# hyeeiin/ECG-Multimodal-Model

Measured on AMD Instinct MI355X. Metric: samples/sec fwd+bwd, batch-256 multimodal (img+sig+clin), 1->8 MI355X, higher is better.
Workload: dtype bf16; 1 GPU; full multimodal (image 3x224x224 + 5000-pt signal + 16-dim clinical), fwd+bwd+Adam, encoders unfrozen; image_hw=224x224, per_gpu_batch=256, global_batch=256, parallelism=dp1

## Files before the change

### ecg-multimodal-model_amd/csrc/api.hip

```cpp
#include <stdarg.h>

#include "ops.h"

static thread_local char g_err[512] = "";

void ecg_set_error(const char* fmt, ...) {
  va_list ap;
  va_start(ap, fmt);
  vsnprintf(g_err, sizeof(g_err), fmt, ap);
  va_end(ap);
}

static inline ConvGeom geom_of(const ecgmm_conv_desc* c) {
  return make_geom(c->N, c->H, c->W, c->Cin, c->Cout, c->R, c->S, c->stride, c->pad_h, c->pad_w);
}
#define S_(x) ((hipStream_t)(x))

extern "C" {

int ecgmm_version(void) { return ECGMM_VERSION; }
const char* ecgmm_last_error(void) { return g_err; }

const char* ecgmm_switch_name(int i) { return i >= 0 && i < sw::COUNT ? sw::ALL[i]->env : nullptr; }
int ecgmm_switch_get(const char* env_name, int64_t* value) {
// ... 251 lines not shown
  if (c->N < 1 || c->H < 1 || c->W < 1 || c->Cin < 1 || c->Cout < 1 || c->R < 1 || c->S < 1 || c->stride < 1 ||
      c->pad_h < 0 || c->pad_w < 0 || c->H + 2 * c->pad_h < c->R || c->W + 2 * c->pad_w < c->S)
    ECG_FAIL(ECGMM_ERR_SHAPE, "conv_fwd_fused: bad geometry");
  return ecg_conv_igemm(dtype, 0, geom_of(c), x, w_fwd, y, bias, addend, nullptr, act, S_(stream));
}
int ecgmm_fold_conv_bn(int dtype, int layout, const float* w, const float* conv_bias, const float* gamma, const float* beta,
                       const float* running_mean, const float* running_var, float eps, void* w_out, float* b_out,
                       float* scale_out, int Cout, int Cin, int RS, void* stream) {
  if (layout != 0 && layout != 1) ECG_FAIL(ECGMM_ERR_SHAPE, "fold_conv_bn: layout %d (0 = forward pack, 1 = stem pack)", layout);
  EcgFoldItem it = {};
  it.kind = layout == 1 ? ECG_FOLD_STEM : ECG_FOLD_CONV;
  it.w = w; it.conv_bias = conv_bias; it.gamma = gamma; it.beta = beta; it.rm = running_mean; it.rv = running_var;
  it.wout = w_out; it.bout = b_out; it.scale_out = scale_out; it.Cout = Cout; it.Cin = Cin; it.RS = RS;
  return ecg_fold_batch(dtype, &it, 1, eps, S_(stream));
}
int ecgmm_relu_maxpool(int dtype, const void* y, void* out, int N, int H, int W, int C, void* stream) {
  return ecg_relu_maxpool(dtype, y, out, N, H, W, C, S_(stream));
}
int ecgmm_gate_res_relu(int dtype, const void* y, const float* gate, const void* res, void* out, int64_t M, int C,
                        int rows_per_sample, void* stream) {
  return ecg_gate_res_relu(dtype, y, gate, res, out, (long)M, C, rows_per_sample, S_(stream));
}

int ecgmm_avgpool(int dtype, const void* x, float* out, int N, int R, int C, const float* coef, void* stream) {
  return ecg_avgpool(dtype, x, out, N, R, C, coef, S_(stream));
}
int ecgmm_bcast_rows(int dtype, const float* v, void* out, int N, int R, int C, float scale, void* stream) {
  return ecg_bcast_rows(dtype, v, out, N, R, C, scale, S_(stream));
}
int ecgmm_se_gate_grad(int dtype, const void* dout, const void* maskref, const void* y, const float* coef, float* dg,
                       int N, int R, int C, void* stream) {
  return ecg_se_gate_grad(dtype, dout, maskref, y, coef, dg, N, R, C, S_(stream));
}

static int se_mlp_shape(const char* what, int N, int C, int CR) {
  if (N < 1 || C < 1 || C > 1024 || CR < 1 || CR > 64)
    ECG_FAIL(ECGMM_ERR_SHAPE, "%s: N=%d C=%d CR=%d outside N >= 1, C 1..1024, CR 1..64", what, N, C, CR);
  return 0;
}
int ecgmm_se_mlp_fwd(const float* m, const float* w1, const float* b1, const float* w2, const float* b2, float* h, float* g,
                     int N, int C, int CR, void* stream) {
  ECG_TRY(se_mlp_shape("se_mlp_fwd", N, C, CR));
  return ecg_se_mlp_fwd(m, w1, b1, w2, b2, h, g, N, C, CR, S_(stream));
}
int ecgmm_se_mlp_bwd(const float* dg, const float* g, const float* h, const float* m, const float* w1, const float* w2,
                     float* ds, float* dh, float* dm, float* dw1, float* db1, float* dw2, float* db2, int N, int C, int CR,
                     float scale, void* stream) {
  ECG_TRY(se_mlp_shape("se_mlp_bwd", N, C, CR));
  return ecg_se_mlp_bwd(dg, g, h, m, w1, w2, ds, dh, dm, dw1, db1, dw2, db2, N, C, CR, scale, S_(stream));
}

int ecgmm_linear_fwd(const float* x, const float* w, const float* bias, float* y, int B, int In, int Out, int act,
                     void* stream) {
  return ecg_linear_fwd(x, w, bias, y, B, In, Out, act, nullptr, S_(stream));
}
size_t ecgmm_linear_bwd_scratch(int B, int In, int Out) { return ecg_linear_bwd_scratch(B, In, Out); }
int ecgmm_linear_bwd(const float* dz, const float* x, const float* w, float* dx, float* dw, float* db, int B, int In,
                     int Out, void* scratch, size_t scratch_bytes, void* stream) {
  return ecg_linear_bwd(dz, x, w, dx, dw, db, B, In, Out, scratch, scratch_bytes, S_(stream));
}
int ecgmm_act_bwd(const float* dy, const float* y, float* dz, int64_t n, int act, void* stream) {
  return ecg_act_bwd(dy, y, dz, (long)n, act, S_(stream));
}

int ecgmm_layernorm_fwd(const float* const* seg, const int* dims, int nseg, const float* fusion_w, const float* gamma,
                        const float* beta, float* out, float* stat, float* soft_w, int B, float eps, void* stream) {
// ... 98 lines not shown
```

### ecg-multimodal-model_amd/csrc/elementwise.hip

```cpp
#include "ops.h"

namespace {

constexpr int EW_THREADS = 256;

__device__ __forceinline__ u32x4 ld16(const void* p) { return *reinterpret_cast<const u32x4*>(p); }
__device__ __forceinline__ u32x4 ld16s(const void* p) {
#ifndef EW_NO_NT
  return __builtin_nontemporal_load(reinterpret_cast<const u32x4*>(p));
#else
  return *reinterpret_cast<const u32x4*>(p);
#endif
}
struct RowDiv { unsigned mul, sh; };
__device__ __forceinline__ long row_div(long r, RowDiv d) { return (long)(((unsigned long long)(unsigned)r * d.mul) >> d.sh); }
static RowDiv make_row_div(int d) {
  unsigned dd = d < 1 ? 1u : (unsigned)d;
  int l = 0;
  while ((1u << l) < dd) ++l;
  RowDiv r;
  r.mul = (unsigned)(((1ull << (31 + l)) + dd - 1) / dd);
  r.sh = 31u + (unsigned)l;
  return r;
}
// ... 673 lines not shown
    if (dgamma) dgamma[c] = (float)s2;
    if (dbeta) dbeta[c] = (float)s1;
    bcoef[c] = (gamma ? gamma[c] : 1.f) * coef[3 * C + c];
    bcoef[C + c] = (float)(s1 / count);
    bcoef[2 * C + c] = (float)(s2 / count);
  }
}

__global__ __launch_bounds__(1024) void rows_sum_kernel(const float* __restrict__ partial, int rows, int C, float* out,
                                                        int accumulate) {
  __shared__ double sh[16][64];
  const int c = blockIdx.x * 64 + (threadIdx.x & 63);
  const int slice = threadIdx.x >> 6;
  double s = 0.0;
  if (c < C) {
    int r = slice;
    for (; r + 48 < rows; r += 64) {
      float a[4];
#pragma unroll
      for (int u = 0; u < 4; ++u) a[u] = partial[(size_t)(r + 16 * u) * C + c];
#pragma unroll
      for (int u = 0; u < 4; ++u) s += (double)a[u];
    }
    for (; r < rows; r += 16) s += (double)partial[(size_t)r * C + c];
  }
  sh[slice][threadIdx.x & 63] = s;
  __syncthreads();
  if (slice == 0 && c < C) {
    for (int k = 1; k < 16; ++k) s += sh[k][threadIdx.x];
    out[c] = accumulate ? out[c] + (float)s : (float)s;
  }
}

template <typename T>
__global__ __launch_bounds__(EW_THREADS) void bnrelu_maxpool_kernel(const T* __restrict__ y,
                                                                    const float* __restrict__ coef, T* __restrict__ out,
                                                                    unsigned char* __restrict__ idx, int N, int H,
                                                                    int W, int C, int OH, int OW) {
  constexpr int VEC = Elem<T>::VEC;
  const int cpr = C / VEC;
  long total = (long)N * OH * OW * cpr;
  for (long i = (long)blockIdx.x * blockDim.x + threadIdx.x; i < total; i += (long)gridDim.x * blockDim.x) {
    int chunk = (int)(i % cpr);
    long pix = i / cpr;
    int ow = (int)(pix % OW);
    long t = pix / OW;
    int oh = (int)(t % OH), n = (int)(t / OH);
    int c0 = chunk * VEC;
    float best[VEC];
    int bi[VEC];
    if constexpr (sizeof(T) == 2) {
      unsigned key[VEC];
      float scv[VEC], shv[VEC];
#pragma unroll
      for (int j = 0; j < VEC; ++j) {
        key[j] = 0u;
        scv[j] = coef[c0 + j];
        shv[j] = coef[C + c0 + j];
      }
#pragma unroll
      for (int kh = 0; kh < 3; ++kh) {
        int h = oh * 2 - 1 + kh;
        if ((unsigned)h >= (unsigned)H) continue;
#pragma unroll
        for (int kw = 0; kw < 3; ++kw) {
          int w = ow * 2 - 1 + kw;
          if ((unsigned)w >= (unsigned)W) continue;
          float f[VEC];
          unpack16<T>(ld16(y + (((size_t)n * H + h) * W + w) * C + c0), f);
#pragma unroll
          for (int j = 0; j < VEC; ++j) f[j] = fmaxf(f[j] * scv[j] + shv[j], 0.f);
          const u32x4 r = pack16<bf16_t>(f);
          const unsigned tcode = 15u - (unsigned)(kh * 3 + kw);
#pragma unroll
          for (int q = 0; q < 4; ++q) {
            key[2 * q] = max(key[2 * q], ((r[q] & 0x7fffu) << 4) | tcode);
            key[2 * q + 1] = max(key[2 * q + 1], (((r[q] >> 16) & 0x7fffu) << 4) | tcode);
          }
        }
      }
#pragma unroll
      for (int j = 0; j < VEC; ++j) {
        best[j] = __uint_as_float((key[j] >> 4) << 16);
        bi[j] = 15 - (int)(key[j] & 15u);
      }
    } else {
#pragma unroll
      for (int j = 0; j < VEC; ++j) {
        best[j] = -INFINITY;
        bi[j] = 0;
      }
#pragma unroll
      for (int kh = 0; kh < 3; ++kh) {
        int h = oh * 2 - 1 + kh;
        if ((unsigned)h >= (unsigned)H) continue;
#pragma unroll
        for (int kw = 0; kw < 3; ++kw) {
          int w = ow * 2 - 1 + kw;
          if ((unsigned)w >= (unsigned)W) continue;
          float f[VEC];
          unpack16<T>(ld16(y + (((size_t)n * H + h) * W + w) * C + c0), f);
#pragma unroll
          for (int j = 0; j < VEC; ++j) {
            float a = fmaxf(f[j] * coef[c0 + j] + coef[C + c0 + j], 0.f);
            if (a > best[j]) {
              best[j] = a;
              bi[j] = kh * 3 + kw;
            }
          }
        }
      }
    }
    st16(out + pix * C + c0, pack16<T>(best));
    unsigned pk[VEC / 4];
#pragma unroll
    for (int q = 0; q < VEC / 4; ++q)
      pk[q] = (unsigned)bi[4 * q] | ((unsigned)bi[4 * q + 1] << 8) | ((unsigned)bi[4 * q + 2] << 16) |
              ((unsigned)bi[4 * q + 3] << 24);
    unsigned* ip = reinterpret_cast<unsigned*>(idx + pix * C + c0);
    if constexpr (VEC == 8) *reinterpret_cast<uint2*>(ip) = make_uint2(pk[0], pk[1]);
    else ip[0] = pk[0];
  }
}

template <typename T>
__global__ __launch_bounds__(EW_THREADS) void maxpool_relu_bwd_kernel(const T* __restrict__ dp,
                                                                      const T* __restrict__ pooled,
                                                                      const unsigned char* __restrict__ idx,
                                                                      T* __restrict__ dz, int N, int H, int W, int C,
                                                                      int OH, int OW) {
  constexpr int VEC = Elem<T>::VEC;
  const int cpr = C / VEC;
  const int H2 = (H + 1) >> 1, W2 = (W + 1) >> 1;
  long total = (long)N * H2 * W2 * cpr;
  for (long i = (long)blockIdx.x * blockDim.x + threadIdx.x; i < total; i += (long)gridDim.x * blockDim.x) {
    int chunk = (int)(i % cpr);
    long blk = i / cpr;
    int m = (int)(blk % W2);
    long t = blk / W2;
    int k = (int)(t % H2), n = (int)(t / H2);
    int c0 = chunk * VEC;
    float d[4][VEC], pv[4][VEC];
    unsigned pk[4][2];
    bool wok[4];
#pragma unroll
    for (int a = 0; a < 2; ++a)
#pragma unroll
      for (int b = 0; b < 2; ++b) {
        const int q = a * 2 + b;
        wok[q] = k + a < OH && m + b < OW;
        const size_t o = (((size_t)n * OH + (wok[q] ? k + a : k)) * OW + (wok[q] ? m + b : m)) * C + c0;
        unpack16<T>(ld16(dp + o), d[q]);
        unpack16<T>(ld16(pooled + o), pv[q]);
        if constexpr (VEC == 8) {
// ... 178 lines not shown
  }
  if (partial) {
#pragma unroll
    for (int j = 0; j < VEC; ++j) shm[threadIdx.x][j] = a1[j];
    __syncthreads();
    for (int c = threadIdx.x; c < C; c += POOL_THREADS) {
      int ck = c / VEC, j = c % VEC;
      float sum = 0.f;
      for (int k = 0; k < bpi; ++k) sum += shm[k * cpr + ck][j];
      partial[(size_t)blockIdx.x * C + c] = sum;
    }
  }
}

template <typename T, bool SEGATE>
__global__ __launch_bounds__(EW_THREADS) void sample_reduce_kernel(const T* __restrict__ x,
                                                                   const T* __restrict__ maskref,
                                                                   const T* __restrict__ y,
                                                                   const float* __restrict__ coef,
                                                                   float* __restrict__ out, int R, int C) {
  constexpr int VEC = Elem<T>::VEC;
  __shared__ float sh[EW_THREADS][VEC + 1];
  const int cpr = C / VEC, nsl = EW_THREADS / cpr;
  const int chunk = threadIdx.x % cpr, slice = threadIdx.x / cpr;
  const int n = blockIdx.x, c0 = chunk * VEC;
  float acc[VEC], sc[VEC], sf[VEC];
#pragma unroll
  for (int j = 0; j < VEC; ++j) {
    acc[j] = 0.f;
    sc[j] = (SEGATE || coef) ? coef[c0 + j] : 1.f;
    sf[j] = (SEGATE || coef) ? coef[C + c0 + j] : 0.f;
  }
  int r = slice;
  if (!SEGATE) {
    for (; r + 3 * nsl < R; r += 4 * nsl) {
      u32x4 q[4];
#pragma unroll
      for (int u = 0; u < 4; ++u) q[u] = ld16(x + ((size_t)n * R + r + u * nsl) * C + c0);
#pragma unroll
      for (int u = 0; u < 4; ++u) {
        float f[VEC];
        unpack16<T>(q[u], f);
#pragma unroll
        for (int j = 0; j < VEC; ++j) acc[j] += f[j];
      }
    }
  }
  for (; r < R; r += nsl) {
    const size_t o = ((size_t)n * R + r) * C + c0;
    float f[VEC];
    unpack16<T>(ld16(x + o), f);
    if (SEGATE) {
      float m[VEC], v[VEC];
      unpack16<T>(ld16(maskref + o), m);
      unpack16<T>(ld16(y + o), v);
#pragma unroll
      for (int j = 0; j < VEC; ++j)
        if (m[j] > 0.f) acc[j] += f[j] * (v[j] * sc[j] + sf[j]);
    } else {
#pragma unroll
      for (int j = 0; j < VEC; ++j) acc[j] += f[j];
    }
  }
#pragma unroll
  for (int j = 0; j < VEC; ++j) sh[threadIdx.x][j] = acc[j];
  __syncthreads();
  for (int c = threadIdx.x; c < C; c += EW_THREADS) {
    const int ck = c / VEC, j = c % VEC;
    float s_ = 0.f;
    for (int k = 0; k < nsl; ++k) s_ += sh[k * cpr + ck][j];
    if (!SEGATE) {
      s_ /= (float)R;
      if (coef) s_ = s_ * coef[c] + coef[C + c];
    }
    out[(size_t)n * C + c] = s_;
  }
}

template <typename T>
__global__ __launch_bounds__(EW_THREADS) void se_gate_bn_kernel(const T* __restrict__ dout, const T* __restrict__ maskref,
                                                                const T* __restrict__ y, const float* __restrict__ coef,
                                                                T* __restrict__ dz, float* __restrict__ dg,
                                                                float* __restrict__ a1o, float* __restrict__ a2o,
                                                                float* __restrict__ a3o, int R, int C) {
  constexpr int VEC = Elem<T>::VEC;
  __shared__ float sh[EW_THREADS][VEC + 1];
  const int cpr = C / VEC, nsl = EW_THREADS / cpr;
  const int chunk = threadIdx.x % cpr, slice = threadIdx.x / cpr;
  const int n = blockIdx.x, c0 = chunk * VEC;
  float sc[VEC], sf[VEC], mu[VEC], ag[VEC], a1[VEC], a2[VEC], a3[VEC];
#pragma unroll
  for (int j = 0; j < VEC; ++j) {
    sc[j] = coef[c0 + j];
    sf[j] = coef[C + c0 + j];
    mu[j] = coef[2 * C + c0 + j];
    ag[j] = a1[j] = a2[j] = a3[j] = 0.f;
  }
  for (int r = slice; r < R; r += nsl) {
    const size_t o = ((size_t)n * R + r) * C + c0;
    float f[VEC], m[VEC], v[VEC];
    unpack16<T>(ld16(dout + o), f);
    unpack16<T>(ld16(maskref + o), m);
    unpack16<T>(ld16(y + o), v);
#pragma unroll
    for (int j = 0; j < VEC; ++j) {
      f[j] = m[j] > 0.f ? f[j] : 0.f;
      const float yc = v[j] - mu[j];
      ag[j] += f[j] * (v[j] * sc[j] + sf[j]);
      a1[j] += f[j];
      a2[j] += f[j] * yc;
      a3[j] += yc;
    }
    st16(dz + o, pack16<T>(f));
  }
  float* const outs[4] = {dg, a1o, a2o, a3o};
#pragma unroll
  for (int q = 0; q < 4; ++q) {
#pragma unroll
    for (int j = 0; j < VEC; ++j) sh[threadIdx.x][j] = q == 0 ? ag[j] : q == 1 ? a1[j] : q == 2 ? a2[j] : a3[j];
    __syncthreads();
    for (int c = threadIdx.x; c < C; c += EW_THREADS) {
      const int ck = c / VEC, j = c % VEC;
      float s_ = 0.f;
      for (int k = 0; k < nsl; ++k) s_ += sh[k * cpr + ck][j];
      outs[q][(size_t)n * C + c] = s_;
    }
    __syncthreads();
  }
}

constexpr int SE_ROWS = 16;
__global__ __launch_bounds__(256) void se_bn_rows_kernel(const float* __restrict__ a1, const float* __restrict__ a2,
                                                         const float* __restrict__ a3, const float* __restrict__ gate,
                                                         const float* __restrict__ addc, int N, int R, int C,
                                                         float* __restrict__ rows) {
  __shared__ float sh[2][4][64];
  const int c = blockIdx.x * 64 + (threadIdx.x & 63), sl = threadIdx.x >> 6, j = blockIdx.y;
  float s1 = 0.f, s2 = 0.f;
  if (c < C)
    for (int n = j + SE_ROWS * sl; n < N; n += SE_ROWS * 4) {
      const size_t o = (size_t)n * C + c;
      const float g = gate ? gate[o] : 1.f, ad = addc ? addc[o] : 0.f;
      s1 += g * a1[o] + ad * (float)R;
      s2 += g * a2[o] + ad * a3[o];
    }
  sh[0][sl][threadIdx.x & 63] = s1;
// ... 492 lines not shown
  hipLaunchKernelGGL(bn_bwd_finalize_kernel, dim3(ceil_div(C, 64)), dim3(1024), 0, stream, (const float*)partial, g1, C,
                     (double)M, gamma, coef, dgamma, dbeta, bcoef, 1);
  ECG_CHECK_LAUNCH("bn_bwd_finalize");
  *bcoef_out = bcoef;
  return 0;
}

bool ecg_stem_fuse_on() { return sw::STEM_FUSE.get() != 0; }

int ecg_pool_bn_bwd(int dtype, const void* dp, const void* pooled, const unsigned char* idx, const void* y,
                    const float* coef, const float* gamma, float* dgamma, float* dbeta, void* dy, float* dbias, int N,
                    int H, int W, int C, float* scratch, hipStream_t stream) {
  if (!chunk_ok(C, dtype)) ECG_FAIL(ECGMM_ERR_SHAPE, "pool_bn_bwd: C=%d unsupported", C);
  const int OH = (H - 1) / 2 + 1, OW = (W - 1) / 2 + 1;
  const int rows = bn_bwd_rows(dtype, (long)N * H * W, C);
  DISPATCH_T(dtype, (pool_bwd_launch<bf16_t>(dp, pooled, idx, y, coef, gamma, dgamma, dbeta, dy, dbias, N, H, W, C, OH, OW, scratch, rows, stream)),
             (pool_bwd_launch<float>(dp, pooled, idx, y, coef, gamma, dgamma, dbeta, dy, dbias, N, H, W, C, OH, OW, scratch, rows, stream)),
             "pool_bn_bwd");
  ECG_CHECK_LAUNCH("pool_bn_bwd");
  return 0;
}

int ecg_rows_sum(const float* partial, int rows, int C, float* out, int accumulate, hipStream_t stream) {
  hipLaunchKernelGGL(rows_sum_kernel, dim3(ceil_div(C, 64)), dim3(1024), 0, stream, partial, rows, C, out, accumulate);
  ECG_CHECK_LAUNCH("rows_sum");
  return 0;
}

int ecg_bnrelu_maxpool(int dtype, const void* y, const float* coef, void* out, unsigned char* idx, int N, int H, int W,
                       int C, hipStream_t stream) {
  if (!chunk_ok(C, dtype)) ECG_FAIL(ECGMM_ERR_SHAPE, "maxpool: C=%d unsupported", C);
  int OH = (H + 2 - 3) / 2 + 1, OW = (W + 2 - 3) / 2 + 1;
  int vec = dtype == ECGMM_BF16 ? 8 : 4;
  int grid = ew_grid((long)N * OH * OW * (C / vec), EW_THREADS);
  DISPATCH_T(dtype,
             hipLaunchKernelGGL(bnrelu_maxpool_kernel<bf16_t>, dim3(grid), dim3(EW_THREADS), 0, stream,
                                (const bf16_t*)y, coef, (bf16_t*)out, idx, N, H, W, C, OH, OW),
             hipLaunchKernelGGL(bnrelu_maxpool_kernel<float>, dim3(grid), dim3(EW_THREADS), 0, stream, (const float*)y,
                                coef, (float*)out, idx, N, H, W, C, OH, OW),
             "maxpool");
  ECG_CHECK_LAUNCH("bnrelu_maxpool");
  return 0;
}

int ecg_maxpool_relu_bwd(int dtype, const void* dp, const void* pooled, const unsigned char* idx, void* dz, int N,
                         int H, int W, int C, hipStream_t stream) {
  if (!chunk_ok(C, dtype)) ECG_FAIL(ECGMM_ERR_SHAPE, "maxpool bwd: C=%d unsupported", C);
  int OH = (H + 2 - 3) / 2 + 1, OW = (W + 2 - 3) / 2 + 1;
  int vec = dtype == ECGMM_BF16 ? 8 : 4;
  int grid = ew_grid((long)N * ((H + 1) / 2) * ((W + 1) / 2) * (C / vec), EW_THREADS);
  DISPATCH_T(dtype,
             hipLaunchKernelGGL(maxpool_relu_bwd_kernel<bf16_t>, dim3(grid), dim3(EW_THREADS), 0, stream,
                                (const bf16_t*)dp, (const bf16_t*)pooled, idx, (bf16_t*)dz, N, H, W, C, OH, OW),
             hipLaunchKernelGGL(maxpool_relu_bwd_kernel<float>, dim3(grid), dim3(EW_THREADS), 0, stream,
                                (const float*)dp, (const float*)pooled, idx, (float*)dz, N, H, W, C, OH, OW),
             "maxpool bwd");
  ECG_CHECK_LAUNCH("maxpool_relu_bwd");
  return 0;
}

int ecg_avgpool(int dtype, const void* x, float* out, int N, int R, int C, const float* coef, hipStream_t stream) {
  if (!chunk_ok(C, dtype)) ECG_FAIL(ECGMM_ERR_SHAPE, "avgpool: C=%d unsupported", C);
  DISPATCH_T(dtype,
             hipLaunchKernelGGL((sample_reduce_kernel<bf16_t, false>), dim3(N), dim3(EW_THREADS), 0, stream,
                                (const bf16_t*)x, (const bf16_t*)nullptr, (const bf16_t*)nullptr, coef, out, R, C),
             hipLaunchKernelGGL((sample_reduce_kernel<float, false>), dim3(N), dim3(EW_THREADS), 0, stream,
                                (const float*)x, (const float*)nullptr, (const float*)nullptr, coef, out, R, C),
// ... 136 lines not shown
```

### ecg-multimodal-model_amd/hip/lib.py

```python
import ctypes as C
import os

F32, BF16 = 0, 1
ACT_NONE, ACT_RELU, ACT_SIGMOID = 0, 1, 2
RESNET18_NPARAMS, RESNET18_NBUFFERS = 62, 60
RESNET1D_NPARAMS, RESNET1D_NBUFFERS = 52, 27

_PKG_DIR = os.path.dirname(os.path.dirname(os.path.abspath(__file__)))
LIB_PATH = os.environ.get("ECGMM_LIB") or os.path.join(_PKG_DIR, "libecgmm_hip.so")

vp, i32, i64, u64, f32, f64, sz = C.c_void_p, C.c_int, C.c_int64, C.c_uint64, C.c_float, C.c_double, C.c_size_t


class ConvDesc(C.Structure):
    _fields_ = [(n, i32) for n in ("N", "H", "W", "Cin", "Cout", "R", "S", "stride", "pad_h", "pad_w")]


class ResNet18Desc(C.Structure):
    _fields_ = [("N", i32), ("H", i32), ("W", i32), ("out_dim", i32), ("dtype", i32), ("training", i32),
                ("bn_momentum", f32), ("bn_eps", f32)]


class ResNet1DDesc(C.Structure):
    _fields_ = [("N", i32), ("cin", i32), ("L", i32), ("num_classes", i32), ("dtype", i32), ("training", i32),
# ... 81 lines not shown
    "ecgmm_stem_bwd_weight_workspace": (sz, [i32, i32, i32, i32, i32]),
    "ecgmm_stem_bwd_weight": (i32, [i32, vp, vp, vp, i32, vp, sz, i32, i32, i32, i32, i32, vp]),
    "ecgmm_stem_bwd_data": (i32, [i32, vp, vp, vp, i32, i32, i32, i32, i32, vp]),
    "ecgmm_col_stats_rows": (i32, [i32, i64, i32]),
    "ecgmm_col_stats": (i32, [i32, vp, i64, i32, vp, vp]),
    "ecgmm_bn_finalize": (i32, [vp, i32, i32, f64, vp, vp, vp, vp, vp, f32, f32, vp, vp]),
    "ecgmm_bn_eval_coef": (i32, [i32, vp, vp, vp, vp, f32, vp, vp]),
    "ecgmm_bn_act": (i32, [i32, vp, vp, vp, vp, vp, i32, i32, vp, i64, i32, vp]),
    "ecgmm_bn_act_from_rows": (i32, [i32, vp, vp, i32, f64, vp, vp, vp, vp, vp, f32, f32, vp, vp, vp, vp, i32, i32, vp, i64, i32, vp]),
    "ecgmm_bn_bwd_scratch": (sz, [i32, i64, i32]),
    "ecgmm_bn_bwd": (i32, [i32, vp, vp, vp, vp, i32, vp, vp, vp, vp, vp, vp, vp, vp, i64, i32, vp, vp]),
    "ecgmm_bn_eval_bwd": (i32, [i32, vp, vp, vp, vp, i32, vp, vp, vp, vp, vp, vp, vp, i64, i32, vp, vp]),
    "ecgmm_conv_bwd_data_with_downsample": (i32, [i32, P(ConvDesc), vp, vp, vp, vp, vp, vp, vp]),
    "ecgmm_conv_bwd_data_bnred": (i32, [i32, P(ConvDesc), vp, vp, vp, vp, vp, vp, vp, vp, P(i32), vp]),
    "ecgmm_conv_bwd_data_bnred_rows": (i32, [i32, P(ConvDesc)]),
    "ecgmm_bn_bwd_from_rows": (i32, [i32, vp, vp, vp, vp, vp, vp, vp, vp, vp, i32, i64, i32, vp, vp]),
    "ecgmm_bnrelu_maxpool": (i32, [i32, vp, vp, vp, vp, i32, i32, i32, i32, vp]),
    "ecgmm_maxpool_relu_bwd": (i32, [i32, vp, vp, vp, vp, i32, i32, i32, i32, vp]),
    "ecgmm_bn_fuse_min_pixels": (i32, [i64]),
    "ecgmm_bn_fold": (i32, [i32]),
    "ecgmm_bn_fold_slice": (i32, [i32]),
    "ecgmm_bn_act_from_rows_bits": (i32, [i32, vp, vp, i32, f64, vp, vp, vp, vp, vp, f32, f32, vp, vp, vp, vp, i32, i32, vp, vp, i64, i32, vp]),
    "ecgmm_bn_bwd_bits": (i32, [i32, vp, vp, vp, vp, i32, vp, vp, vp, vp, vp, vp, vp, vp, i64, i32, vp, vp]),
    "ecgmm_bn_bwd_dual": (i32, [i32] + [vp] * 19 + [i64, i32, vp, vp, vp]),
    "ecgmm_bn_dual": (i32, [i32]),
    "ecgmm_tl_enable": (i32, [i32]),
    "ecgmm_tl_mark": (i32, [i32, vp]),
    "ecgmm_tl_collect": (i32, [i32, vp, vp]),
    "ecgmm_stem_recompute": (i32, [i32]),
    "ecgmm_pool_bn_bwd": (i32, [i32, vp, vp, vp, vp, vp, vp, vp, vp, vp, vp, i32, i32, i32, i32, vp, vp]),
    "ecgmm_avgpool": (i32, [i32, vp, vp, i32, i32, i32, vp, vp]),
    "ecgmm_bcast_rows": (i32, [i32, vp, vp, i32, i32, i32, f32, vp]),
    "ecgmm_se_gate_grad": (i32, [i32, vp, vp, vp, vp, vp, i32, i32, i32, vp]),
    "ecgmm_se_mlp_fwd": (i32, [vp, vp, vp, vp, vp, vp, vp, i32, i32, i32, vp]),
    "ecgmm_se_mlp_bwd": (i32, [vp, vp, vp, vp, vp, vp, vp, vp, vp, vp, vp, vp, vp, i32, i32, i32, f32, vp]),
    "ecgmm_linear_fwd": (i32, [vp, vp, vp, vp, i32, i32, i32, i32, vp]),
    "ecgmm_linear_bwd_scratch": (sz, [i32, i32, i32]),
    "ecgmm_linear_bwd": (i32, [vp, vp, vp, vp, vp, vp, i32, i32, i32, vp, sz, vp]),
    "ecgmm_act_bwd": (i32, [vp, vp, vp, i64, i32, vp]),
    "ecgmm_layernorm_fwd": (i32, [P(vp), P(i32), i32, vp, vp, vp, vp, vp, vp, i32, f32, vp]),
    "ecgmm_layernorm_bwd_scratch": (sz, [i32, i32]),
    "ecgmm_layernorm_bwd": (i32, [P(vp), P(i32), i32, vp, vp, vp, vp, P(vp), i32, vp, vp, vp, i32, vp, vp]),
    "ecgmm_varloss_fwd": (i32, [vp, vp, vp, i32, i32, i32, i32, vp, vp, vp]),
    "ecgmm_varloss_bwd": (i32, [vp, i32, i32, vp, vp, i32, vp, i32, vp]),
    "ecgmm_ce_fwd": (i32, [vp, vp, i32, i32, i32, f32, f32, vp, vp, vp]),
    "ecgmm_ce_bwd": (i32, [vp, vp, i32, i32, vp, vp, vp, vp]),
    "ecgmm_ce_plus_fwd": (i32, [vp, vp, i32, i32, vp, f32, vp, vp, vp]),
    "ecgmm_ce_plus_bwd": (i32, [vp, vp, i32, i32, vp, vp, vp, vp, f32, vp]),
    "ecgmm_dropout_fwd": (i32, [vp, vp, vp, i64, f32, u64, u64, vp]),
    "ecgmm_dropout_bwd": (i32, [vp, vp, vp, i64, f32, vp]),
    "ecgmm_adam": (i32, [vp, vp, vp, vp, i64, f32, f32, f32, f32, f32, i64, f32, vp]),
    "ecgmm_axpby": (i32, [f32, vp, f32, vp, i64, vp]),
    "ecgmm_signal_preprocess_workspace": (sz, [i32, i32, i32]),
    "ecgmm_signal_preprocess": (i32, [vp, vp, i32, i32, vp, vp, i32, P(f64), P(f64), P(f64), i32, vp, sz, vp]),
    "ecgmm_signal_preprocess_i16": (i32, [vp, i32, i32, i32, P(i32), i32, vp, vp, i32, vp, i32, i32, P(f64), P(f64), P(f64),
                                          i32, vp]),
    "ecgmm_weighted_sample": (i32, [vp, i64, i64, vp, vp, i64, u64, u64, vp]),
    "ecgmm_signal_filter_zscore": (i32, [vp, vp, i32, i32, P(f64), P(f64), P(f64), i32, i32, f64, vp]),
    "ecgmm_signal_gather_augment": (i32, [vp, i64, i32, vp, i32, vp, vp, i32, f32, f32, f32, f32, i32, i32, u64, u64, vp]),
    "ecgmm_glu_fwd": (i32, [vp, vp, i64, i32, vp]),
    "ecgmm_glu_bwd": (i32, [vp, vp, vp, i64, i32, vp]),
    "ecgmm_sparsemax_fwd": (i32, [vp, vp, i64, i32, vp]),
    "ecgmm_sparsemax_bwd": (i32, [vp, vp, vp, i64, i32, vp]),
    "ecgmm_ew": (i32, [i32, vp, vp, vp, i64, f32, vp]),
    "ecgmm_split_cols": (i32, [vp, vp, vp, i64, i32, i32, i32, vp]),
    "ecgmm_split_cols_bwd": (i32, [vp, vp, vp, vp, i64, i32, i32, i32, vp]),
# ... 48 lines not shown
    "ecgmm_shap_gradient": (i32, [vp, vp, vp, vp, vp, vp, vp, i32, i32, i32, i32, i32, i32, vp, vp, vp, vp, sz, vp]),
    "ecgmm_shap_deep": (i32, [vp, vp, vp, vp, vp, i32, i32, i32, i32, i32, vp, vp, vp, vp, sz, vp]),
    "ecgmm_mha_bwd_workspace": (sz, [P(MHADesc)]),
    "ecgmm_mha_forward": (i32, [P(MHADesc), vp, vp, vp, u64, u64, vp]),
    "ecgmm_mha_backward": (i32, [P(MHADesc), vp, vp, vp, vp, vp, vp, sz, u64, u64, vp]),
    "ecgmm_mha_keep_mask": (i32, [P(MHADesc), vp, u64, u64, vp]),
    "ecgmm_embed1d_fwd": (i32, [vp, vp, vp, vp, vp, i32, i32, i32, i32, vp]),
    "ecgmm_embed1d_bwd_workspace": (sz, [i32, i32, i32, i32]),
    "ecgmm_embed1d_bwd": (i32, [vp, vp, vp, vp, vp, vp, vp, i32, i32, i32, i32, i32, vp, sz, vp]),
}

LATER_SYMBOLS = ("ecgmm_resnet18_backward_dx", "ecgmm_resnet18_gradcam", "ecgmm_resnet1d_backward_dx",
                 "ecgmm_resnet1d_gradcam", "ecgmm_stem_bwd_data", "ecgmm_bn_eval_bwd", "ecgmm_bn_small_eval_bwd",
                 "ecgmm_resnet18_infer_prepared_bytes", "ecgmm_resnet18_infer_prepare", "ecgmm_resnet18_infer_workspace",
                 "ecgmm_resnet18_infer", "ecgmm_resnet1d_infer_prepared_bytes", "ecgmm_resnet1d_infer_prepare",
                 "ecgmm_resnet1d_infer_workspace", "ecgmm_resnet1d_infer", "ecgmm_infer_down_side", "ecgmm_conv_fwd_fused",
                 "ecgmm_fold_conv_bn", "ecgmm_relu_maxpool", "ecgmm_gate_res_relu",
                 "ecgmm_signal_filter_zscore", "ecgmm_signal_gather_augment",
                 "ecgmm_lstm_fwd_workspace", "ecgmm_lstm_bwd_workspace", "ecgmm_lstm_forward", "ecgmm_lstm_backward",
                 "ecgmm_conv5_in1_stats_rows", "ecgmm_conv5_in1_fwd", "ecgmm_conv5_in1_bwd_weight_workspace",
                 "ecgmm_conv5_in1_bwd_weight", "ecgmm_conv5_bwd_weight_workspace", "ecgmm_conv5_bwd_weight",
                 "ecgmm_bnrelu_maxpool2", "ecgmm_pool2_bn_bwd_workspace", "ecgmm_pool2_bn_bwd",
                 "ecgmm_crnn_front_fwd_workspace", "ecgmm_crnn_front_bwd_workspace", "ecgmm_crnn_front_forward",
                 "ecgmm_crnn_front_backward",
                 "ecgmm_switch_name", "ecgmm_switch_get", "ecgmm_switch_set",
                 "ecgmm_log_spectrogram_frames", "ecgmm_log_spectrogram",
                 "ecgmm_se_mlp_fwd", "ecgmm_se_mlp_bwd",
                 "ecgmm_signal_preprocess_i16", "ecgmm_weighted_sample",
                 "ecgmm_resnet18_ws_view", "ecgmm_resnet1d_ws_view",
                 "ecgmm_lime_perturb", "ecgmm_lime_ridge_workspace", "ecgmm_lime_ridge", "ecgmm_lime_prob",
                 "ecgmm_shap_mlp_workspace", "ecgmm_shap_gradient", "ecgmm_shap_deep",
                 "ecgmm_bn_bwd_dual", "ecgmm_bn_dual",
                 "ecgmm_mha_bwd_workspace", "ecgmm_mha_forward", "ecgmm_mha_backward", "ecgmm_mha_keep_mask",
                 "ecgmm_embed1d_fwd", "ecgmm_embed1d_bwd_workspace", "ecgmm_embed1d_bwd")

_lib = None


def _missing(name):
    def fail(*_a):
        raise RuntimeError(f"{LIB_PATH} does not export {name}: rebuild the HIP library (there is no fallback)")
    return fail


def lib():
    global _lib
    if _lib is None:
        if not os.path.exists(LIB_PATH):
            raise RuntimeError(
                f"libecgmm_hip.so not found at {LIB_PATH}: the HIP extension is the only compute path "
                "(no CPU fallback). Build it with `python __graft_entry__.py` or "
                "`make -C ecg-multimodal-model_amd/csrc`.")
        import torch
        h = C.CDLL(LIB_PATH)
        for name, (res, args) in SIGNATURES.items():
            if name in LATER_SYMBOLS and os.environ.get("ECGMM_LIB") and not hasattr(h, name):
                setattr(h, name, _missing(name))
                continue
            fn = getattr(h, name)
            fn.restype, fn.argtypes = res, args
        if h.ecgmm_version() != 100:
            raise RuntimeError(f"libecgmm_hip.so version {h.ecgmm_version()} != 100 (stale build?)")
        _lib = h
    return _lib


def check(rc, what=""):
# ... 4 lines not shown
```

### include/ecgmm.h

```cpp
#ifndef ECGMM_H
#define ECGMM_H
#include <stddef.h>
#include <stdint.h>

#ifdef __cplusplus
extern "C" {
#endif

#define ECGMM_VERSION 100

enum { ECGMM_F32 = 0, ECGMM_BF16 = 1 };
enum { ECGMM_ACT_NONE = 0, ECGMM_ACT_RELU = 1, ECGMM_ACT_SIGMOID = 2 };
enum {
  ECGMM_OK = 0,
  ECGMM_ERR_SHAPE = 1,
  ECGMM_ERR_DTYPE = 2,
  ECGMM_ERR_WORKSPACE = 3,
  ECGMM_ERR_LAUNCH = 4
};

int ecgmm_version(void);
const char* ecgmm_last_error(void);

const char* ecgmm_switch_name(int i);
// ... 179 lines not shown
                           const float* gamma, float* dgamma, float* dbeta, void* dy, const float* rows, int nrows,
                           int64_t M, int C, void* scratch, void* stream);

int ecgmm_bn_fuse_min_pixels(int64_t m);
int ecgmm_bn_fold(int on);
int ecgmm_bn_fold_slice(int on);
int ecgmm_bn_act_from_rows_bits(int dtype, const void* y, const float* partial, int rows, double count, const float* gamma,
                                const float* beta, float* running_mean, float* running_var, int64_t* num_batches_tracked,
                                float momentum, float eps, float* coef_out, const void* res, const float* rcoef,
                                const float* gate, int rows_per_sample, int relu, void* out, uint8_t* relu_bits, int64_t M,
                                int C, void* stream);
int ecgmm_bn_bwd_bits(int dtype, const void* dout, const uint8_t* mask_bits, const float* gate, const float* addc,
                      int rows_per_sample, const void* y, const float* coef, const float* gamma, float* dgamma,
                      float* dbeta, void* dy, void* dz_out, float* dbias, int64_t M, int C, void* scratch, void* stream);
int ecgmm_bn_bwd_dual(int dtype, const void* dout, const void* maskref, const uint8_t* mask_bits, const float* gate,
                      const float* addc, const void* y_a, const float* coef_a, const float* gamma_a, float* dgamma_a,
                      float* dbeta_a, void* dy_a, const void* y_b, const float* coef_b, const float* gamma_b,
                      float* dgamma_b, float* dbeta_b, void* dy_b, void* dz, float* dbias, int64_t M, int C, void* scratch_a,
                      void* scratch_b, void* stream);
int ecgmm_bn_dual(int on);
int ecgmm_stem_recompute(int on);

int ecgmm_bnrelu_maxpool(int dtype, const void* y, const float* coef, void* out, uint8_t* idx, int N, int H, int W,
                         int C, void* stream);
int ecgmm_maxpool_relu_bwd(int dtype, const void* dp, const void* pooled, const uint8_t* idx, void* dz, int N, int H,
                           int W, int C, void* stream);
int ecgmm_pool_bn_bwd(int dtype, const void* dp, const void* pooled, const uint8_t* idx, const void* y, const float* coef,
                      const float* gamma, float* dgamma, float* dbeta, void* dy, float* dbias, int N, int H, int W, int C,
                      void* scratch, void* stream);
int ecgmm_avgpool(int dtype, const void* x, float* out, int N, int R, int C, const float* coef, void* stream);
int ecgmm_bcast_rows(int dtype, const float* v, void* out, int N, int R, int C, float scale, void* stream);
int ecgmm_se_gate_grad(int dtype, const void* dout, const void* maskref, const void* y, const float* coef, float* dg,
                       int N, int R, int C, void* stream);
int ecgmm_se_mlp_fwd(const float* m, const float* w1, const float* b1, const float* w2, const float* b2, float* h, float* g,
                     int N, int C, int CR, void* stream);
int ecgmm_se_mlp_bwd(const float* dg, const float* g, const float* h, const float* m, const float* w1, const float* w2,
                     float* ds, float* dh, float* dm, float* dw1, float* db1, float* dw2, float* db2, int N, int C, int CR,
                     float scale, void* stream);

int ecgmm_linear_fwd(const float* x, const float* w, const float* bias, float* y, int B, int In, int Out, int act,
                     void* stream);
size_t ecgmm_linear_bwd_scratch(int B, int In, int Out);
int ecgmm_linear_bwd(const float* dz, const float* x, const float* w, float* dx, float* dw, float* db, int B, int In,
                     int Out, void* scratch, size_t scratch_bytes, void* stream);
int ecgmm_act_bwd(const float* dy, const float* y, float* dz, int64_t n, int act, void* stream);

int ecgmm_layernorm_fwd(const float* const* seg, const int* dims, int nseg, const float* fusion_w, const float* gamma,
                        const float* beta, float* out, float* stat, float* soft_w, int B, float eps, void* stream);
size_t ecgmm_layernorm_bwd_scratch(int B, int D);
int ecgmm_layernorm_bwd(const float* const* seg, const int* dims, int nseg, const float* fusion_w, const float* gamma,
                        const float* stat, const float* dout, float* const* dseg, int dseg_accumulate, float* dgamma,
                        float* dbeta, float* dfusion_w, int B, void* scratch, void* stream);

int ecgmm_varloss_fwd(const float* f0, const float* f1, const float* f2, int B, int D0, int D1, int D2, float* loss,
                      float* scratch, void* stream);
int ecgmm_varloss_bwd(const float* f, int B, int D, const float* gout, const float* scratch, int which, float* df,
                      int accumulate, void* stream);

int ecgmm_ce_fwd(const float* logits, const int64_t* labels, int B, int C, int focal, float alpha, float gamma,
                 float* loss, float* dcoef, void* stream);
int ecgmm_ce_bwd(const float* logits, const int64_t* labels, int B, int C, const float* dcoef, const float* gout,
                 float* dlogits, void* stream);
int ecgmm_ce_plus_fwd(const float* logits, const int64_t* labels, int B, int C, const float* extra, float extra_w,
                      float* loss, float* dcoef, void* stream);
int ecgmm_ce_plus_bwd(const float* logits, const int64_t* labels, int B, int C, const float* dcoef, const float* gout,
                      float* dlogits, float* dextra, float extra_w, void* stream);
// ... 145 lines not shown
```

Baseline: 40000 samples/s.

## Pool two output columns per thread and batch loads in SE gate kernels

The BN+ReLU+maxpool kernel now computes two adjacent output columns per thread from one shared 3x5 window. Overlapping input columns are loaded once, and the window is clamped and masked rather than branched. Per-channel BN coefficients are hoisted out of the grid-stride loop. The SE gate-grad and gate+BN backward kernels are unrolled by four rows with all loads issued before compute, which exposes more memory-level parallelism. A C API entry for the fused se_gate_bn kernel is also exported. Register pressure rises, and hoisting the coefficients assumes the grid stride is a multiple of cpr.

Result: faster. 40680 samples/s, median of 6 (+1.7%).

```diff
diff --git a/ecg-multimodal-model_amd/csrc/api.hip b/ecg-multimodal-model_amd/csrc/api.hip
--- a/ecg-multimodal-model_amd/csrc/api.hip
+++ b/ecg-multimodal-model_amd/csrc/api.hip
@@ -307,6 +307,12 @@
                        int N, int R, int C, void* stream) {
   return ecg_se_gate_grad(dtype, dout, maskref, y, coef, dg, N, R, C, S_(stream));
 }
+int ecgmm_se_gate_bn(int dtype, const void* dout, const void* maskref, const void* y, const float* coef, void* dz, float* dg,
+                     float* a1, float* a2, float* a3, int N, int R, int C, void* stream) {
+  if (!dout || !maskref || !y || !coef || !dz || !dg || !a1 || !a2 || !a3) ECG_FAIL(ECGMM_ERR_SHAPE, "se_gate_bn: null operand");
+  if (N < 1 || R < 1) ECG_FAIL(ECGMM_ERR_SHAPE, "se_gate_bn: N=%d R=%d", N, R);
+  return ecg_se_gate_bn(dtype, dout, maskref, y, coef, dz, dg, a1, a2, a3, N, R, C, S_(stream));
+}
 
 static int se_mlp_shape(const char* what, int N, int C, int CR) {
   if (N < 1 || C < 1 || C > 1024 || CR < 1 || CR > 64)
diff --git a/ecg-multimodal-model_amd/csrc/elementwise.hip b/ecg-multimodal-model_amd/csrc/elementwise.hip
--- a/ecg-multimodal-model_amd/csrc/elementwise.hip
+++ b/ecg-multimodal-model_amd/csrc/elementwise.hip
@@ -729,6 +729,99 @@
   }
 }
 
+template <typename T, int NR>
+__device__ __forceinline__ void pool_window2(const T* __restrict__ y, const float* scv, const float* shv, int n, int oh,
+                                             int ow0, int H, int W, int C, int c0, float (*best)[Elem<T>::VEC],
+                                             int (*bi)[Elem<T>::VEC]) {
+  constexpr int VEC = Elem<T>::VEC;
+  constexpr int KH0 = NR == 1 ? 1 : 0;
+  u32x4 q[NR * 5];
+  bool in[NR * 5];
+#pragma unroll
+  for (int kh = 0; kh < NR; ++kh) {
+    const int h = oh * 2 - 1 + KH0 + kh;
+    const int hc = min(max(h, 0), H - 1);
+#pragma unroll
+    for (int c = 0; c < 5; ++c) {
+      const int w = ow0 * 2 - 1 + c;
+      const int wc = min(max(w, 0), W - 1);
+      in[kh * 5 + c] = h == hc && w == wc;
+      q[kh * 5 + c] = ld16(y + (((size_t)n * H + hc) * W + wc) * C + c0);
+    }
+  }
+  __builtin_amdgcn_sched_barrier(0);
+  if constexpr (sizeof(T) == 2) {
+    unsigned key[2][VEC];
+#pragma unroll
+    for (int j = 0; j < VEC; ++j) key[0][j] = key[1][j] = 0u;
+#pragma unroll
+    for (int kh = 0; kh < NR; ++kh) {
+#pragma unroll
+      for (int c = 0; c < 5; ++c) {
+        const int t = kh * 5 + c;
+        float f[VEC];
+        unpack16<T>(q[t], f);
+#pragma unroll
+        for (int j = 0; j < VEC; ++j) f[j] = fmaxf(f[j] * scv[j] + shv[j], 0.f);
+        const u32x4 r = pack16<bf16_t>(f);
+        const unsigned m = in[t] ? 0x7fffu : 0u;
+        const unsigned tc0 = in[t] ? 15u - (unsigned)((KH0 + kh) * 3 + c) : 0u;
+        const unsigned tc1 = in[t] ? 15u - (unsigned)((KH0 + kh) * 3 + c - 2) : 0u;
+#pragma unroll
+        for (int k = 0; k < 4; ++k) {
+          const unsigned lo = (r[k] & m) << 4, hi = ((r[k] >> 16) & m) << 4;
+          if (c <= 2) {
+            key[0][2 * k] = max(key[0][2 * k], lo | tc0);
+            key[0][2 * k + 1] = max(key[0][2 * k + 1], hi | tc0);
+          }
+          if (c >= 2) {
+            key[1][2 * k] = max(key[1][2 * k], lo | tc1);
+            key[1][2 * k + 1] = max(key[1][2 * k + 1], hi | tc1);
+          }
+        }
+      }
+    }
+#pragma unroll
+    for (int o = 0; o < 2; ++o) {
+#pragma unroll
+      for (int j = 0; j < VEC; ++j) {
+        best[o][j] = __uint_as_float((key[o][j] >> 4) << 16);
+        bi[o][j] = 15 - (int)(key[o][j] & 15u);
+      }
+    }
+  } else {
+#pragma unroll
+    for (int o = 0; o < 2; ++o) {
+#pragma unroll
+      for (int j = 0; j < VEC; ++j) {
+        best[o][j] = -INFINITY;
+        bi[o][j] = 0;
+      }
+    }
+#pragma unroll
+    for (int kh = 0; kh < NR; ++kh) {
+#pragma unroll
+      for (int c = 0; c < 5; ++c) {
+        const int t = kh * 5 + c;
+        float f[VEC];
+        unpack16<T>(q[t], f);
+#pragma unroll
+        for (int j = 0; j < VEC; ++j) {
+          float a = fmaxf(f[j] * scv[j] + shv[j], 0.f);
+          if (c <= 2 && in[t] && a > best[0][j]) {
+            best[0][j] = a;
+            bi[0][j] = (KH0 + kh) * 3 + c;
+          }
+          if (c >= 2 && in[t] && a > best[1][j]) {
+            best[1][j] = a;
+            bi[1][j] = (KH0 + kh) * 3 + c - 2;
+          }
+        }
+      }
+    }
+  }
+}
+
 template <typename T>
 __global__ __launch_bounds__(EW_THREADS) void bnrelu_maxpool_kernel(const T* __restrict__ y,
                                                                     const float* __restrict__ coef, T* __restrict__ out,
@@ -736,87 +829,38 @@
                                                                     int W, int C, int OH, int OW) {
   constexpr int VEC = Elem<T>::VEC;
   const int cpr = C / VEC;
-  long total = (long)N * OH * OW * cpr;
+  const int OWP = (OW + 1) / 2;
+  long total = (long)N * OH * OWP * cpr;
+  const int c0 = (int)(((long)blockIdx.x * blockDim.x + threadIdx.x) % cpr) * VEC;
+  float scv[VEC], shv[VEC];
+#pragma unroll
+  for (int j = 0; j < VEC; ++j) {
+    scv[j] = coef[c0 + j];
+    shv[j] = coef[C + c0 + j];
+  }
   for (long i = (long)blockIdx.x * blockDim.x + threadIdx.x; i < total; i += (long)gridDim.x * blockDim.x) {
-    int chunk = (int)(i % cpr);
-    long pix = i / cpr;
-    int ow = (int)(pix % OW);
-    long t = pix / OW;
+    long pp = i / cpr;
+    int ow0 = (int)(pp % OWP) * 2;
+    long t = pp / OWP;
     int oh = (int)(t % OH), n = (int)(t / OH);
-    int c0 = chunk * VEC;
-    float best[VEC];
-    int bi[VEC];
-    if constexpr (sizeof(T) == 2) {
-      unsigned key[VEC];
-      float scv[VEC], shv[VEC];
-#pragma unroll
-      for (int j = 0; j < VEC; ++j) {
-        key[j] = 0u;
-        scv[j] = coef[c0 + j];
-        shv[j] = coef[C + c0 + j];
-      }
-#pragma unroll
-      for (int kh = 0; kh < 3; ++kh) {
-        int h = oh * 2 - 1 + kh;
-        if ((unsigned)h >= (unsigned)H) continue;
-#pragma unroll
-        for (int kw = 0; kw < 3; ++kw) {
-          int w = ow * 2 - 1 + kw;
-          if ((unsigned)w >= (unsigned)W) continue;
-          float f[VEC];
-          unpack16<T>(ld16(y + (((size_t)n * H + h) * W + w) * C + c0), f);
-#pragma unroll
-          for (int j = 0; j < VEC; ++j) f[j] = fmaxf(f[j] * scv[j] + shv[j], 0.f);
-          const u32x4 r = pack16<bf16_t>(f);
-          const unsigned tcode = 15u - (unsigned)(kh * 3 + kw);
-#pragma unroll
-          for (int q = 0; q < 4; ++q) {
-            key[2 * q] = max(key[2 * q], ((r[q] & 0x7fffu) << 4) | tcode);
-            key[2 * q + 1] = max(key[2 * q + 1], (((r[q] >> 16) & 0x7fffu) << 4) | tcode);
-          }
-        }
-      }
-#pragma unroll
-      for (int j = 0; j < VEC; ++j) {
-        best[j] = __uint_as_float((key[j] >> 4) << 16);
-        bi[j] = 15 - (int)(key[j] & 15u);
-      }
-    } else {
-#pragma unroll
-      for (int j = 0; j < VEC; ++j) {
-        best[j] = -INFINITY;
-        bi[j] = 0;
-      }
-#pragma unroll
-      for (int kh = 0; kh < 3; ++kh) {
-        int h = oh * 2 - 1 + kh;
-        if ((unsigned)h >= (unsigned)H) continue;
-#pragma unroll
-        for (int kw = 0; kw < 3; ++kw) {
-          int w = ow * 2 - 1 + kw;
-          if ((unsigned)w >= (unsigned)W) continue;
-          float f[VEC];
-          unpack16<T>(ld16(y + (((size_t)n * H + h) * W + w) * C + c0), f);
-#pragma unroll
-          for (int j = 0; j < VEC; ++j) {
-            float a = fmaxf(f[j] * coef[c0 + j] + coef[C + c0 + j], 0.f);
-            if (a > best[j]) {
-              best[j] = a;
-              bi[j] = kh * 3 + kw;
-            }
-          }
-        }
-      }
-    }
-    st16(out + pix * C + c0, pack16<T>(best));
-    unsigned pk[VEC / 4];
-#pragma unroll
-    for (int q = 0; q < VEC / 4; ++q)
-      pk[q] = (unsigned)bi[4 * q] | ((unsigned)bi[4 * q + 1] << 8) | ((unsigned)bi[4 * q + 2] << 16) |
-              ((unsigned)bi[4 * q + 3] << 24);
-    unsigned* ip = reinterpret_cast<unsigned*>(idx + pix * C + c0);
-    if constexpr (VEC == 8) *reinterpret_cast<uint2*>(ip) = make_uint2(pk[0], pk[1]);
-    else ip[0] = pk[0];
+    float best[2][VEC];
+    int bi[2][VEC];
+    if (H == 1) pool_window2<T, 1>(y, scv, shv, n, oh, ow0, H, W, C, c0, best, bi);
+    else pool_window2<T, 3>(y, scv, shv, n, oh, ow0, H, W, C, c0, best, bi);
+    const long pix = ((long)n * OH + oh) * OW + ow0;
+#pragma unroll
+    for (int o = 0; o < 2; ++o) {
+      if (ow0 + o >= OW) break;
+      st16(out + (pix + o) * C + c0, pack16<T>(best[o]));
+      unsigned pk[VEC / 4];
+#pragma unroll
+      for (int q = 0; q < VEC / 4; ++q)
+        pk[q] = (unsigned)bi[o][4 * q] | ((unsigned)bi[o][4 * q + 1] << 8) | ((unsigned)bi[o][4 * q + 2] << 16) |
+                ((unsigned)bi[o][4 * q + 3] << 24);
+      unsigned* ip = reinterpret_cast<unsigned*>(idx + (pix + o) * C + c0);
+      if constexpr (VEC == 8) *reinterpret_cast<uint2*>(ip) = make_uint2(pk[0], pk[1]);
+      else ip[0] = pk[0];
+    }
   }
 }
 
@@ -1061,7 +1105,28 @@
     sf[j] = (SEGATE || coef) ? coef[C + c0 + j] : 0.f;
   }
   int r = slice;
-  if (!SEGATE) {
+  if (SEGATE) {
+    for (; r + 3 * nsl < R; r += 4 * nsl) {
+      u32x4 q[4], qm[4], qv[4];
+#pragma unroll
+      for (int u = 0; u < 4; ++u) {
+        const size_t o = ((size_t)n * R + r + u * nsl) * C + c0;
+        q[u] = ld16(x + o);
+        qm[u] = ld16(maskref + o);
+        qv[u] = ld16(y + o);
+      }
+#pragma unroll
+      for (int u = 0; u < 4; ++u) {
+        float f[VEC], m[VEC], v[VEC];
+        unpack16<T>(q[u], f);
+        unpack16<T>(qm[u], m);
+        unpack16<T>(qv[u], v);
+#pragma unroll
+        for (int j = 0; j < VEC; ++j)
+          if (m[j] > 0.f) acc[j] += f[j] * (v[j] * sc[j] + sf[j]);
+      }
+    }
+  } else {
     for (; r + 3 * nsl < R; r += 4 * nsl) {
       u32x4 q[4];
 #pragma unroll
@@ -1077,16 +1142,19 @@
   }
   for (; r < R; r += nsl) {
     const size_t o = ((size_t)n * R + r) * C + c0;
-    float f[VEC];
-    unpack16<T>(ld16(x + o), f);
+    const u32x4 q = ld16(x + o);
     if (SEGATE) {
-      float m[VEC], v[VEC];
-      unpack16<T>(ld16(maskref + o), m);
-      unpack16<T>(ld16(y + o), v);
+      const u32x4 qm = ld16(maskref + o), qv = ld16(y + o);
+      float f[VEC], m[VEC], v[VEC];
+      unpack16<T>(q, f);
+      unpack16<T>(qm, m);
+      unpack16<T>(qv, v);
 #pragma unroll
       for (int j = 0; j < VEC; ++j)
         if (m[j] > 0.f) acc[j] += f[j] * (v[j] * sc[j] + sf[j]);
     } else {
+      float f[VEC];
+      unpack16<T>(q, f);
 #pragma unroll
       for (int j = 0; j < VEC; ++j) acc[j] += f[j];
     }
@@ -1125,12 +1193,11 @@
     mu[j] = coef[2 * C + c0 + j];
     ag[j] = a1[j] = a2[j] = a3[j] = 0.f;
   }
-  for (int r = slice; r < R; r += nsl) {
-    const size_t o = ((size_t)n * R + r) * C + c0;
+  auto row = [&](size_t o, const u32x4& qd, const u32x4& qm, const u32x4& qv) __attribute__((always_inline)) {
     float f[VEC], m[VEC], v[VEC];
-    unpack16<T>(ld16(dout + o), f);
-    unpack16<T>(ld16(maskref + o), m);
-    unpack16<T>(ld16(y + o), v);
+    unpack16<T>(qd, f);
+    unpack16<T>(qm, m);
+    unpack16<T>(qv, v);
 #pragma unroll
     for (int j = 0; j < VEC; ++j) {
       f[j] = m[j] > 0.f ? f[j] : 0.f;
@@ -1141,6 +1208,25 @@
       a3[j] += yc;
     }
     st16(dz + o, pack16<T>(f));
+  };
+  int r = slice;
+  for (; r + 3 * nsl < R; r += 4 * nsl) {
+    u32x4 qd[4], qm[4], qv[4];
+#pragma unroll
+    for (int u = 0; u < 4; ++u) {
+      const size_t o = ((size_t)n * R + r + u * nsl) * C + c0;
+      qd[u] = ld16(dout + o);
+      qm[u] = ld16(maskref + o);
+      qv[u] = ld16(y + o);
+    }
+    __builtin_amdgcn_sched_barrier(0);
+#pragma unroll
+    for (int u = 0; u < 4; ++u) row(((size_t)n * R + r + u * nsl) * C + c0, qd[u], qm[u], qv[u]);
+  }
+  for (; r < R; r += nsl) {
+    const size_t o = ((size_t)n * R + r) * C + c0;
+    const u32x4 qd = ld16(dout + o), qm = ld16(maskref + o), qv = ld16(y + o);
+    row(o, qd, qm, qv);
   }
   float* const outs[4] = {dg, a1o, a2o, a3o};
 #pragma unroll
@@ -1699,7 +1785,7 @@
   if (!chunk_ok(C, dtype)) ECG_FAIL(ECGMM_ERR_SHAPE, "maxpool: C=%d unsupported", C);
   int OH = (H + 2 - 3) / 2 + 1, OW = (W + 2 - 3) / 2 + 1;
   int vec = dtype == ECGMM_BF16 ? 8 : 4;
-  int grid = ew_grid((long)N * OH * OW * (C / vec), EW_THREADS);
+  int grid = ew_grid((long)N * OH * ((OW + 1) / 2) * (C / vec), EW_THREADS);
   DISPATCH_T(dtype,
              hipLaunchKernelGGL(bnrelu_maxpool_kernel<bf16_t>, dim3(grid), dim3(EW_THREADS), 0, stream,
                                 (const bf16_t*)y, coef, (bf16_t*)out, idx, N, H, W, C, OH, OW),
diff --git a/ecg-multimodal-model_amd/hip/lib.py b/ecg-multimodal-model_amd/hip/lib.py
--- a/ecg-multimodal-model_amd/hip/lib.py
+++ b/ecg-multimodal-model_amd/hip/lib.py
@@ -137,6 +137,7 @@
     "ecgmm_avgpool": (i32, [i32, vp, vp, i32, i32, i32, vp, vp]),
     "ecgmm_bcast_rows": (i32, [i32, vp, vp, i32, i32, i32, f32, vp]),
     "ecgmm_se_gate_grad": (i32, [i32, vp, vp, vp, vp, vp, i32, i32, i32, vp]),
+    "ecgmm_se_gate_bn": (i32, [i32, vp, vp, vp, vp, vp, vp, vp, vp, vp, i32, i32, i32, vp]),
     "ecgmm_se_mlp_fwd": (i32, [vp, vp, vp, vp, vp, vp, vp, i32, i32, i32, vp]),
     "ecgmm_se_mlp_bwd": (i32, [vp, vp, vp, vp, vp, vp, vp, vp, vp, vp, vp, vp, vp, i32, i32, i32, f32, vp]),
     "ecgmm_linear_fwd": (i32, [vp, vp, vp, vp, i32, i32, i32, i32, vp]),
@@ -251,7 +252,8 @@
                  "ecgmm_shap_mlp_workspace", "ecgmm_shap_gradient", "ecgmm_shap_deep",
                  "ecgmm_bn_bwd_dual", "ecgmm_bn_dual",
                  "ecgmm_mha_bwd_workspace", "ecgmm_mha_forward", "ecgmm_mha_backward", "ecgmm_mha_keep_mask",
-                 "ecgmm_embed1d_fwd", "ecgmm_embed1d_bwd_workspace", "ecgmm_embed1d_bwd")
+                 "ecgmm_embed1d_fwd", "ecgmm_embed1d_bwd_workspace", "ecgmm_embed1d_bwd",
+                 "ecgmm_se_gate_bn")
 
 _lib = None
 
diff --git a/include/ecgmm.h b/include/ecgmm.h
--- a/include/ecgmm.h
+++ b/include/ecgmm.h
@@ -235,6 +235,8 @@
 int ecgmm_bcast_rows(int dtype, const float* v, void* out, int N, int R, int C, float scale, void* stream);
 int ecgmm_se_gate_grad(int dtype, const void* dout, const void* maskref, const void* y, const float* coef, float* dg,
                        int N, int R, int C, void* stream);
+int ecgmm_se_gate_bn(int dtype, const void* dout, const void* maskref, const void* y, const float* coef, void* dz, float* dg,
+                     float* a1, float* a2, float* a3, int N, int R, int C, void* stream);
 int ecgmm_se_mlp_fwd(const float* m, const float* w1, const float* b1, const float* w2, const float* b2, float* h, float* g,
                      int N, int C, int CR, void* stream);
 int ecgmm_se_mlp_bwd(const float* dg, const float* g, const float* h, const float* m, const float* w1, const float* w2,
```
